# roryclear/clearcam

Hardware: AMD Instinct MI355X
Metric: yolov9c_640x640_frames_per_sec (higher is better)
Workload: dtype f16; 1 GPU; YOLOv9-C f16h batch=64 640x640 frames (letterbox 640) per GPU, uint8 BGR frames resident in HBM, seeded synthetic weights, full detect path (letterbox+convs+decode+top300+NMS); batch_per_gpu=64, parallelism=one camera batch per GPU x1, no collective, batches_in_flight=3

## Files before the change

clearcam_amd/csrc/conv_direct.hip:

```cpp
#include "kernels.h"

namespace cc {

template <class T>
__global__ __launch_bounds__(256) void conv_direct_kernel(const ConvP p) {
  const size_t total = (size_t)p.B * p.Ho * p.Wo * p.Cout;
  const size_t idx = (size_t)blockIdx.x * 256 + threadIdx.x;
  if (idx >= total) return;
  const int n = (int)(idx % p.Cout);
  const size_t m = idx / p.Cout;
  const int hw = p.Ho * p.Wo;
  const int b = (int)(m / hw), rem = (int)(m - (size_t)b * hw), ho = rem / p.Wo, wo = rem - ho * p.Wo;
  const T* w = reinterpret_cast<const T*>(p.w) + (size_t)n * p.Kw;
  float acc = 0.f;
  for (int r = 0; r < p.ks; ++r) {
    const int ih = ho * p.stride - p.pad + r;
    if ((unsigned)ih >= (unsigned)p.Hin) continue;
    for (int s = 0; s < p.ks; ++s) {
      const int iw = wo * p.stride - p.pad + s;
      if ((unsigned)iw >= (unsigned)p.Win) continue;
      for (int h = 0; h <= p.split; ++h) {
        const T* wk = w + ((r * p.ks + s) * (1 + p.split) + h) * p.Cin;
        {
          const Src& S = p.s0;
// ... 159 lines not shown

template <class T>
__global__ __launch_bounds__(256) void avgmax_rows2_kernel(const PoolP p) {
  constexpr int E = 16 / (int)sizeof(T);
  const int CV = p.C / E;
  const int x = blockIdx.x * 256 + threadIdx.x;
  if (x >= p.Wo * CV) return;
  const int wo = x / CV, cv = x - wo * CV, ho0 = blockIdx.y * 2, b = blockIdx.z;
  const T* in = reinterpret_cast<const T*>(p.in) + p.in_coff + cv * E;
  const int i0 = 2 * ho0 - 1, j0 = 2 * wo - 1;
  uint4 u[6][4];
#pragma unroll
  for (int r = 0; r < 6; ++r) {
    const int ic = min(max(i0 + r, 0), p.H - 1);
#pragma unroll
    for (int c = 0; c < 4; ++c) {
      const int jc = min(max(j0 + c, 0), p.W - 1);
      u[r][c] = *reinterpret_cast<const uint4*>(in + ((size_t)(b * p.H + ic) * p.W + jc) * p.in_cstride);
    }
  }
#pragma unroll
  for (int q = 0; q < 2; ++q) {
    const int ho = ho0 + q;
    if (ho >= p.Ho) break;
    float acc[E];
#pragma unroll
    for (int e = 0; e < E; ++e) acc[e] = -INFINITY;
#pragma unroll
    for (int r = 0; r < 3; ++r) {
      const int ph = i0 + 2 * q + r;
      float top[4][E], bot[4][E];
#pragma unroll
      for (int c = 0; c < 4; ++c) { unpack_chunk<T>(u[2 * q + r][c], top[c]); unpack_chunk<T>(u[2 * q + r + 1][c], bot[c]); }
#pragma unroll
      for (int s = 0; s < 3; ++s) {
        const int pw = j0 + s;
        const bool ok = ph >= 0 && ph <= p.H - 2 && pw >= 0 && pw <= p.W - 2;
#pragma unroll
        for (int e = 0; e < E; ++e) {
          const float a = (((top[s][e] + top[s + 1][e]) + bot[s][e]) + bot[s + 1][e]) * 0.25f;
          acc[e] = fmaxf(acc[e], ok ? a : -INFINITY);
        }
      }
    }
    uint4 o;
    T* t = reinterpret_cast<T*>(&o);
#pragma unroll
    for (int e = 0; e < E; ++e) t[e] = from_f32<T>(acc[e]);
    const size_t m = ((size_t)b * p.Ho + ho) * p.Wo + wo;
    *reinterpret_cast<uint4*>(reinterpret_cast<T*>(p.out) + m * p.out_cstride + p.out_coff + cv * E) = o;
  }
}

template <class T>
__global__ __launch_bounds__(256) void pool_kernel(const PoolP p) {
  const size_t total = (size_t)p.B * p.Ho * p.Wo * p.C;
  const size_t idx = (size_t)blockIdx.x * 256 + threadIdx.x;
  if (idx >= total) return;
  const int c = (int)(idx % p.C);
  const size_t m = idx / p.C;
  const int hw = p.Ho * p.Wo;
  const int b = (int)(m / hw), rem = (int)(m - (size_t)b * hw), ho = rem / p.Wo, wo = rem - ho * p.Wo;
  const T* in = reinterpret_cast<const T*>(p.in);
  float acc = p.mode ? -INFINITY : 0.f;
  for (int r = 0; r < p.k; ++r) {
    const int ih = ho * p.stride - p.pad + r;
    if ((unsigned)ih >= (unsigned)p.H) continue;
    for (int s = 0; s < p.k; ++s) {
      const int iw = wo * p.stride - p.pad + s;
      if ((unsigned)iw >= (unsigned)p.W) continue;
      const float v = to_f32<T>(in[((size_t)(b * p.H + ih) * p.W + iw) * p.in_cstride + p.in_coff + c]);
      acc = p.mode ? fmaxf(acc, v) : acc + v;
    }
  }
  if (!p.mode) acc = acc * (1.0f / (float)(p.k * p.k));
  reinterpret_cast<T*>(p.out)[m * p.out_cstride + p.out_coff + c] = from_f32<T>(acc);
}

std::atomic<int> g_pool_rows_override{-1};
constexpr int kNoPoolRows = INT32_MIN;
static int pool_rows() {
  const int ov = g_pool_rows_override.load();
  if (ov >= 0) return ov;
  static const int env = [] { const char* e = getenv("CLEARCAM_POOL_ROWS"); return e ? atoi(e) : kNoPoolRows; }();
  return env;
}

PoolKernel choose_pool(int dt, const PoolP& p) {
  const int E = dt == F32 ? 4 : 8;
  const bool vec = p.C % E == 0 && p.in_coff % E == 0 && p.in_cstride % E == 0 && p.out_coff % E == 0 && p.out_cstride % E == 0 &&
                   ((uintptr_t)p.in & 15) == 0 && ((uintptr_t)p.out & 15) == 0;
  const int set = pool_rows();
  if (p.mode == 2) {
    CC_CHECK(vec && p.k == 3 && p.stride == 2 && p.pad == 1, "avg-max pool: needs 16-byte channel chunks, k=3 s=2 p=1");
    const int rows2 = set == kNoPoolRows ? 4 : set;
    return rows2 != 1 && p.Ho >= 32 ? POOL_AVGMAX_ROWS2 : POOL_AVGMAX;
  }
  if (vec && p.mode == 0 && p.k == 2) {
    const int rows = set == kNoPoolRows ? 8 : set;
    const bool plain = p.stride == 1 && p.pad == 0 && p.Ho >= 64 && p.Wo == p.W - 1 && p.Ho == p.H - 1;
    if (rows == 8 && plain) return POOL_AVG2_ROWS8;
    if (rows == 4 && plain) return POOL_AVG2_ROWS4;
    return POOL_VEC_AVG2;
  }
  if (vec && p.mode == 1 && p.k == 1) return POOL_VEC_MAX1;
  if (vec && p.mode == 1 && p.k == 2) return POOL_VEC_MAX2;
  if (vec && p.mode == 1 && p.k == 3) return POOL_VEC_MAX3;
  if (vec && p.mode == 1 && p.k == 5) return POOL_VEC_MAX5;
  return POOL_SCALAR;
}

template <class T> static void launch_pool_t(PoolKernel k, const PoolP& p, hipStream_t stream) {
  constexpr int E = 16 / (int)sizeof(T);
  const dim3 vgrid((unsigned)((p.Wo * (p.C / E) + 255) / 256), (unsigned)p.Ho, (unsigned)p.B);
  auto rows_grid = [&](int r) { return dim3(vgrid.x, (unsigned)((p.Ho + r - 1) / r), vgrid.z); };
  switch (k) {
    case POOL_AVGMAX_ROWS2: hipLaunchKernelGGL(avgmax_rows2_kernel<T>, rows_grid(2), dim3(256), 0, stream, p); break;
    case POOL_AVGMAX: hipLaunchKernelGGL(avgmax_pool_kernel<T>, vgrid, dim3(256), 0, stream, p); break;
    case POOL_AVG2_ROWS8: hipLaunchKernelGGL((avg2_rows_kernel<T, 8>), rows_grid(8), dim3(256), 0, stream, p); break;
    case POOL_AVG2_ROWS4: hipLaunchKernelGGL((avg2_rows_kernel<T, 4>), rows_grid(4), dim3(256), 0, stream, p); break;
    case POOL_VEC_AVG2: hipLaunchKernelGGL((pool_vec_kernel<T, 2, 0>), vgrid, dim3(256), 0, stream, p); break;
    case POOL_VEC_MAX1: hipLaunchKernelGGL((pool_vec_kernel<T, 1, 1>), vgrid, dim3(256), 0, stream, p); break;
    case POOL_VEC_MAX2: hipLaunchKernelGGL((pool_vec_kernel<T, 2, 1>), vgrid, dim3(256), 0, stream, p); break;
    case POOL_VEC_MAX3: hipLaunchKernelGGL((pool_vec_kernel<T, 3, 1>), vgrid, dim3(256), 0, stream, p); break;
    case POOL_VEC_MAX5: hipLaunchKernelGGL((pool_vec_kernel<T, 5, 1>), vgrid, dim3(256), 0, stream, p); break;
    case POOL_SCALAR: {
      const size_t total = (size_t)p.B * p.Ho * p.Wo * p.C;
      hipLaunchKernelGGL(pool_kernel<T>, dim3((unsigned)((total + 255) / 256)), dim3(256), 0, stream, p);
      break;
    }
  }
  CC_HIP(hipGetLastError());
}

template <class T>
__global__ __launch_bounds__(256) void fuse_kernel(const FuseP p) {
  constexpr int E = 16 / (int)sizeof(T);
  const int CV = p.C / E;
  const size_t total = (size_t)p.B * p.Ho * p.Wo * CV;
  const size_t idx = (size_t)blockIdx.x * 256 + threadIdx.x;
  if (idx >= total) return;
  const int cv = (int)(idx % CV);
  const size_t m = idx / CV;
  const int hw = p.Ho * p.Wo;
  const int b = (int)(m / hw), rem = (int)(m - (size_t)b * hw), ho = rem / p.Wo, wo = rem - ho * p.Wo;
  float acc[E];
#pragma unroll
  for (int e = 0; e < E; ++e) acc[e] = 0.f;
  for (int k = 0; k < p.n; ++k) {
    const T* in = reinterpret_cast<const T*>(p.in[k]) +
                  ((size_t)(b * p.H[k] + (ho >> p.shift[k])) * p.W[k] + (wo >> p.shift[k])) * p.cstride[k] + p.coff[k] + cv * E;
    const uint4 u = *reinterpret_cast<const uint4*>(in);
    const T* t = reinterpret_cast<const T*>(&u);
#pragma unroll
    for (int e = 0; e < E; ++e) acc[e] += to_f32<T>(t[e]);
  }
  uint4 o;
  T* t = reinterpret_cast<T*>(&o);
#pragma unroll
  for (int e = 0; e < E; ++e) t[e] = from_f32<T>(acc[e]);
  *reinterpret_cast<uint4*>(reinterpret_cast<T*>(p.out) + m * p.out_cstride + p.out_coff + cv * E) = o;
}

void launch_fuse(int dt, const FuseP& p, hipStream_t stream) {
  const int E = dt == F32 ? 4 : 8;
  CC_CHECK(p.C % E == 0 && p.out_coff % E == 0 && p.out_cstride % E == 0, "fuse: channel alignment");
  for (int k = 0; k < p.n; ++k) CC_CHECK(p.coff[k] % E == 0 && p.cstride[k] % E == 0, "fuse: input channel alignment");
  const size_t total = (size_t)p.B * p.Ho * p.Wo * (p.C / E);
  const dim3 grid((unsigned)((total + 255) / 256)), block(256);
// ... 16 lines not shown
```

clearcam_amd/csrc/dev_glue.hip:

```cpp
#include "conv_select.h"
#include "yolo_plan.h"

using namespace cc;

namespace {

bool aligned16(const void* p) { return (reinterpret_cast<uintptr_t>(p) & 15u) == 0; }
constexpr long kMaxElems = 1L << 30;

PoolP pool_args(int dtype, const void* in_dev, int in_cstride, int in_coff, void* out_dev, int out_cstride, int out_coff, int B, int H, int W,
                int C, int Ho, int Wo, int k, int stride, int pad, int mode) {
  CC_CHECK(dtype == F32 || dtype == F16 || dtype == BF16, "dtype must be 0 (f32), 1 (f16) or 2 (bf16)");
  CC_CHECK(in_dev && out_dev, "null argument");
  CC_CHECK(B > 0 && H > 0 && W > 0 && C > 0 && Ho > 0 && Wo > 0, "bad shape");
  CC_CHECK(mode >= 0 && mode <= 2 && k > 0 && k <= 16 && stride > 0 && pad >= 0 && pad < k, "bad window");
  CC_CHECK(in_coff >= 0 && in_coff + C <= in_cstride && out_coff >= 0 && out_coff + C <= out_cstride, "bad channel view");
  CC_CHECK((long)B * H * W * in_cstride < kMaxElems && (long)B * Ho * Wo * out_cstride < kMaxElems, "tensor too large");
  const int Hp = mode == 2 ? H - 1 : H, Wp = mode == 2 ? W - 1 : W;
  CC_CHECK(Hp > 0 && Wp > 0, "avg-max pool: the input needs two rows and two columns");
  if (mode == 0) CC_CHECK(pad == 0 && (Ho - 1) * stride + k <= H && (Wo - 1) * stride + k <= W, "avg pool: windows must lie inside the input (pad 0)");
  else CC_CHECK((Ho - 1) * stride - pad < Hp && (Wo - 1) * stride - pad < Wp, "Ho / Wo beyond the padded input");
  PoolP p{};
  p.in = in_dev; p.in_cstride = in_cstride; p.in_coff = in_coff; p.out = out_dev; p.out_cstride = out_cstride; p.out_coff = out_coff;
  p.B = B; p.H = H; p.W = W; p.C = C; p.Ho = Ho; p.Wo = Wo; p.k = k; p.stride = stride; p.pad = pad; p.mode = mode;
  return p;
}

Src src_view(const cc_src_desc& s) { return Src{s.ptr, s.H, s.W, s.cstride, s.coff, s.C, s.shift}; }

int dev_conv(bool det, bool launch, const cc_conv_desc* d, const cc_src_desc* s0, const cc_src_desc* s1, const float* w_oihw, const float* bias,
             const void* res_dev, void* out_dev, int* choice, void* stream) {
  PackedConv pc;
  auto release = [&]() { if (pc.w) hipFree(pc.w); if (pc.bias) hipFree(pc.bias); pc.w = nullptr; pc.bias = nullptr; };
  try {
    CC_CHECK(d && s0 && out_dev && (w_oihw || !launch), "null argument");
    CC_CHECK(d->dtype == F32 || d->dtype == F16 || d->dtype == BF16 || d->dtype == F16S, "dtype must be 0 (f32), 1 (f16), 2 (bf16) or 3 (f16s)");
    const int split = d->dtype == F16S, dt = storage_dtype(d->dtype);
    CC_CHECK(d->B > 0 && d->H > 0 && d->W > 0 && d->k > 0 && d->k <= 7 && d->stride > 0 && d->Cin > 0 && d->Cout > 0, "bad shape");
    if (!det) CC_CHECK(d->groups == 1 && d->act >= 0 && d->act <= 2 && !d->res_f32 && !d->res_cstride && !d->res_coff, "one group, act 0 .. 2, no residual");
    else {
      CC_CHECK(d->groups >= 1 && d->Cin % d->groups == 0 && d->Cout % d->groups == 0, "groups must divide Cin and Cout");
      CC_CHECK(d->act >= 0 && d->act <= (launch ? 2 : 4), "act 0 .. 2");
      CC_CHECK(res_dev || (!d->res_f32 && !d->res_cstride && !d->res_coff), "a residual view without a residual pointer");
    }
    ConvP c{};
    c.s0 = src_view(*s0);
    c.s1 = s1 ? src_view(*s1) : Src{s0->ptr, 1, 1, 0, 0, 0, 0};
    c.B = d->B; c.Hin = d->H; c.Win = d->W; c.Cin = d->Cin; c.Cout = d->Cout; c.ks = d->k; c.stride = d->stride; c.pad = d->pad < 0 ? d->k / 2 : d->pad;
    c.Ho = d->Ho > 0 ? d->Ho : (c.Hin + 2 * c.pad - c.ks) / c.stride + 1; c.Wo = d->Wo > 0 ? d->Wo : (c.Win + 2 * c.pad - c.ks) / c.stride + 1;
    CC_CHECK(c.s0.C > 0 && c.s1.C >= 0 && c.s0.C + c.s1.C == c.Cin, "Cin must be the channels of the two sources");
    for (const Src* s : {&c.s0, &c.s1}) {
      if (s->C == 0) continue;
      CC_CHECK(s->ptr && s->H > 0 && s->W > 0 && s->coff >= 0 && s->coff + s->C <= s->cstride && (long)c.B * s->H * s->W * s->cstride < kMaxElems, "bad source view");
      CC_CHECK(s->shift >= -1 && s->shift <= 4, "shift must be -1 (2x2 average), 0 or a nearest-upsample exponent");
      if (s->shift >= 0) CC_CHECK(((c.Hin - 1) >> s->shift) < s->H && ((c.Win - 1) >> s->shift) < s->W, "a source is smaller than the input over 2^shift");
      else CC_CHECK(s == &c.s0 && c.Hin == s->H - 1 && c.Win == s->W - 1, "the 2x2 average: first source only, input = (H - 1) x (W - 1) of it");
    }
    c.out = out_dev; c.out_cstride = d->out_cstride > 0 ? d->out_cstride : d->Cout; c.out_coff = d->out_coff; c.out_f32 = d->out_f32 ? 1 : 0;
    c.act = d->act; c.variant = d->variant; c.split = split;
    c.Ktot = c.ks * c.ks * c.Cin * (1 + split);
    c.Kw = (c.Ktot + 63) / 64 * 64;
    CC_CHECK(c.Ho > 0 && c.Wo > 0 && c.out_coff >= 0 && c.out_coff + c.Cout <= c.out_cstride && (long)c.B * c.Ho * c.Wo * c.out_cstride < kMaxElems, "bad output view");
    CC_CHECK(c.pad >= 0 && c.pad < c.ks && (c.Ho - 1) * c.stride - c.pad < c.Hin && (c.Wo - 1) * c.stride - c.pad < c.Win, "Ho / Wo beyond the padded input");
    const bool adown = c.s0.shift < 0;
    if (res_dev) {
      c.res = res_dev; c.res_f32 = d->res_f32 ? 1 : 0; c.res_cstride = d->res_cstride > 0 ? d->res_cstride : d->Cout; c.res_coff = d->res_coff;
      CC_CHECK(c.res_coff >= 0 && c.res_coff + c.Cout <= c.res_cstride && (long)c.B * c.Ho * c.Wo * c.res_cstride < kMaxElems, "bad residual view");
      CC_CHECK(!adown, "the averaging loader takes no residual");
      CC_CHECK(res_dev != out_dev || (c.res_f32 == c.out_f32 && c.res_cstride == c.out_cstride && c.res_coff == c.out_coff),
// ... 93 lines not shown
```

clearcam_amd/csrc/kernels.h:

```cpp
#pragma once
#include <atomic>
#include <vector>
#include "common.h"

namespace cc {

struct LaunchNote { const char* kernel; long tiles; long slots; };
extern thread_local LaunchNote g_launch_note;
extern thread_local bool g_note_launches;
template <class K> inline void note_launch(const char* name, K kernel, long tiles, int threads, size_t lds, long persistent_grid = 0) {
  if (!g_note_launches) return;
  long slots = persistent_grid;
  if (!slots) {
    int nb = 0;
    if (hipOccupancyMaxActiveBlocksPerMultiprocessor(&nb, reinterpret_cast<const void*>(kernel), threads, lds) != hipSuccess) nb = 1;
    slots = (long)nb * cu_count();
  }
  g_launch_note = LaunchNote{name, tiles, slots > 0 ? slots : 1};
}

bool conv_mfma_supported(int dt, const ConvP& p);
void launch_conv_mfma(int dt, const ConvP& p, hipStream_t stream);
void launch_conv_direct(int dt, const ConvP& p, hipStream_t stream);
void launch_conv(int dt, const ConvP& p, hipStream_t stream);
bool conv_adown_supported(int dt, const ConvP& p);
int conv_adown_bn(const ConvP& p);
void launch_conv_adown(int dt, const ConvP& p, hipStream_t stream);

struct CspP {
  const void* x; int x_cstride, x_coff;
  void* out; int out_cstride, out_coff;
  const void* w12; int kw12; const float* b12;
  const void* wr; int kwr; const float* br;
  const void* wb; int kwb; const float* bb;
  const void* w3; int kw3; const float* b3;
  int B, H, W, hid;
  int split; float os12, osr, osb, os3;
  int tx, tiles; float inv_tiles, inv_tx;
  int dbg;
  int stream;
};
bool csp_fused_supported(int dt, int hid, int split = 0);
enum CspKernel : int { CSP_FUSED_RESIDENT = 0, CSP_FUSED_STREAMED = 1, CSP_TILE = 2 };
CspKernel choose_csp(int dt, int hid, int split, int B, int H, int W, int stream, int dbg, int tile_mode);
extern std::atomic<int> g_csp_tile_override;
int csp_tile_mode();
void launch_csp_fused(int dt, const CspP& p, hipStream_t stream, CspKernel* chosen = nullptr);

void launch_sample_rows(const ConvP& p, const int* rows_dev, int S, float* out_dev, hipStream_t stream);
void second_moments(const float* X, int rows, int ci, std::vector<double>& H);
int gptq_round_f16(const float* w, int co, int ci, const double* H, double damp, float* out);

struct PoolP {
  const void* in; int in_cstride, in_coff;
  void* out; int out_cstride, out_coff;
  int B, H, W, C;
  int Ho, Wo;
  int k, stride, pad;
  int mode;
};
enum PoolKernel : int {
  POOL_SCALAR = 0,
  POOL_VEC_MAX1 = 1,
  POOL_VEC_MAX2 = 2,
  POOL_VEC_MAX3 = 3,
  POOL_VEC_MAX5 = 4,
  POOL_VEC_AVG2 = 5,
  POOL_AVG2_ROWS4 = 6,
  POOL_AVG2_ROWS8 = 7,
  POOL_AVGMAX = 8,
  POOL_AVGMAX_ROWS2 = 9,
};
PoolKernel choose_pool(int dt, const PoolP& p);
extern std::atomic<int> g_pool_rows_override;
void launch_pool(int dt, const PoolP& p, hipStream_t stream, PoolKernel* chosen = nullptr);

struct FuseP {
  int n;
  const void* in[6]; int H[6], W[6], cstride[6], coff[6], shift[6];
  void* out; int out_cstride, out_coff;
  int B, Ho, Wo, C;
};
void launch_fuse(int dt, const FuseP& p, hipStream_t stream);

struct PreP {
  const void* frames; int frame_f32;
  int B, H, W;
  int nh, nw, pad_y, pad_x, Hn, Wn;
  const int* xlo; const int* xhi; const float* xfr;
  const int* ylo; const int* yhi; const float* yfr;
  void* out; int out_c;
  int flip;
  float div, sub, pad_val;
};
void launch_preprocess(int dt, const PreP& p, hipStream_t stream);

struct FrameDesc {
  long long off;
  int H, W, nh, nw, pad_y, pad_x;
  const int* xlo; const int* xhi; const float* xfr;
  const int* ylo; const int* yhi; const float* yfr;
  float fpad_x, fpad_y, gain, src_w, src_h;
  int reserved;
};
void launch_preprocess_ragged(int dt, const PreP& p, const FrameDesc* desc, size_t packed_bytes, hipStream_t stream);

struct StemP {
  PreP pre;
  const void* w; const float* bias;
  const void* w_lo; float oscale;
  int Cout;
  void* out; int out_cstride, out_coff;
  int Ho, Wo;
  int abl;
};
bool stem_fused_supported(int dt, int Cout);
void stem_pack_weights(int dt, const void* w_packed, int w_row, int tap_stride, int plane_off, int Cout, void* out, hipStream_t stream);
void launch_stem_fused(int dt, const StemP& p, hipStream_t stream);
bool stem_needs_big(int H, int W, int nh, int nw, int frame_f32);
void launch_stem_fused_ragged(int dt, const StemP& p, const FrameDesc* desc, size_t packed_bytes, bool big, hipStream_t stream);
void axis_tables(int n_in, int n_out, std::vector<int>& lo, std::vector<int>& hi, std::vector<float>& fr);

struct DecodeP {
  const float* raw[3]; int H[3], W[3];
  int B, A;
  const float* dfl_w;
  float conf;
// ... 173 lines not shown
```

clearcam_amd/csrc/yolo.hip:

```cpp
#include <cmath>
#include <cstring>
#include "conv_select.h"
#include "yolo_plan.h"

using namespace cc;

namespace cc {

static const Arch kArch[] = {
    {"t", 16, true, 32, 32, false, 64, 16, 64, 64, 96, 24, 96, 128, 32, 128, 64, 48, 64, 80, 3},
    {"s", 32, true, 64, 64, false, 128, 32, 128, 128, 192, 48, 192, 256, 64, 256, 128, 96, 128, 128, 3},
    {"m", 32, false, 32, 128, false, 240, 60, 240, 240, 360, 90, 360, 480, 120, 480, 240, 184, 240, 240, 1},
    {"c", 64, false, 32, 256, true, 256, 64, 256, 512, 512, 128, 512, 512, 128, 512, 256, 256, 512, 256, 1},
    {"e", 64, false, 32, 256, true, 0, 0, 256, 0, 0, 0, 512, 0, 0, 512, 256, 0, 0, 256, 2},
};

void convert_f32_to(int dt, const float* src, void* dst, size_t n) {
  if (dt == F32) memcpy(dst, src, n * 4);
  else if (dt == F16) { f16_t* d = (f16_t*)dst; for (size_t i = 0; i < n; ++i) d[i] = (f16_t)src[i]; }
  else { uint16_t* d = (uint16_t*)dst; for (size_t i = 0; i < n; ++i) d[i] = f32_to_bf16_bits(src[i]); }
}

static int weight_rounding() {
  static const int mode = [] {
// ... 93 lines not shown
  const int cp = cin_pad > cin ? cin_pad : cin;
  const int planes = split ? 2 : 1;
  const size_t kreal = (size_t)k * k * cp * planes;
  const size_t ktot = (kreal + 63) / 64 * 64;
  std::vector<float> w((size_t)cout * ktot, 0.f), bias(cout, 0.f);
  float scale = 1.0f;
  if (split) {
    float mx = 0.f;
    for (size_t t = 0; t < ws.size(); ++t) for (float v : ws[t]->data) mx = std::max(mx, std::fabs(v));
    if (mx > 0.f && std::isfinite(mx)) scale = std::ldexp(1.0f, 14 - std::ilogb(mx));
    pc.split = 1; pc.oscale = 1.0f / scale;
  }
  int n0 = 0;
  for (size_t t = 0; t < ws.size(); ++t) {
    const int co = (int)ws[t]->shape[0], cig = (int)ws[t]->shape[1], g = groups[t], cog = co / g;
    pc.macs_px += (double)co * cig * k * k;
    std::vector<float> fb;
    if (!split && dt != F32 && weight_rounding() != 0) fb = round_weights(dt, *ws[t]);
    const float* src = fb.empty() ? ws[t]->data.data() : fb.data();
    for (int n = 0; n < co; ++n) {
      const int grp = n / cog;
      for (int c = 0; c < cig; ++c)
        for (int r = 0; r < k; ++r)
          for (int s = 0; s < k; ++s) {
            const float v = src[(((size_t)n * cig + c) * k + r) * k + s];
            float* row = &w[(size_t)(n0 + n) * ktot];
            if (!split) row[(size_t)(r * k + s) * cp + grp * cig + c] = v;
            else {
              const float vs = v * scale;
              const float hi = (float)(f16_t)vs;
              row[(size_t)((r * k + s) * 2 + 0) * cp + grp * cig + c] = hi;
              row[(size_t)((r * k + s) * 2 + 1) * cp + grp * cig + c] = vs - hi;
            }
          }
      if (bs[t]) bias[n0 + n] = bs[t]->data[n];
    }
    n0 += co;
  }
  std::vector<char> tmp(w.size() * dtype_size(dt));
  convert_f32_to(dt, w.data(), tmp.data(), w.size());
  CC_HIP(hipMalloc(&pc.w, tmp.size() + 256));
  CC_HIP(hipMemcpy(pc.w, tmp.data(), tmp.size(), hipMemcpyHostToDevice));
  CC_HIP(hipMalloc((void**)&pc.bias, cout * 4));
  CC_HIP(hipMemcpy(pc.bias, bias.data(), cout * 4, hipMemcpyHostToDevice));
  pc.cin = cp; pc.cout = cout; pc.k = k; pc.kw = (int)ktot;
  return pc;
}

struct PlanSwitches {
  static int num(const char* name, int dflt) { const char* e = getenv(name); return e ? atoi(e) : dflt; }
  static bool set(const char* name) { return getenv(name) != nullptr; }
  const int lanes = num("CLEARCAM_LANES", 0), fuse_csp = num("CLEARCAM_FUSE_CSP", 2);
  const bool fuse_stem = num("CLEARCAM_FUSE_STEM", 1) != 0, fuse_adown = num("CLEARCAM_FUSE_ADOWN", 0) != 0, fuse_head = num("CLEARCAM_FUSE_HEAD", 1) != 0;
  const bool head_split = num("CLEARCAM_HEAD_SPLIT", 1) != 0, arena_reuse = num("CLEARCAM_ARENA_REUSE", 1) != 0;
  const bool tap_csp = set("CLEARCAM_TAP_CSP"), tap_stem = set("CLEARCAM_TAP_STEM"), tap_blocks = set("CLEARCAM_TAP_BLOCKS"), verbose = set("CLEARCAM_VERBOSE");
  const bool dev = num("CLEARCAM_DEV", 0) != 0;
  const bool csp_only_set = dev && set("CLEARCAM_CSP_ONLY");
  const int csp_only = dev ? num("CLEARCAM_CSP_ONLY", 0) : 0, csp_dbg = dev ? num("CLEARCAM_CSP_DBG", 0) : 0, csp_stream = dev ? num("CLEARCAM_CSP_STREAM", 0) : 0;
};

struct Builder {
  cc_yolo* Y; Plan* P; const Arch& a; const PlanSwitches sw;
  Builder(cc_yolo* y, Plan* p) : Y(y), P(p), a(*y->arch) {}

  int cur_lane = 0;
  struct Lane {
    Builder& b; int saved;
    Lane(Builder& b_, int l) : b(b_), saved(b_.cur_lane) {
      const int m = b.sw.lanes;
      if (l == 1 ? (m & 1) : (m & 6)) b.cur_lane = (l > 2 && (m & 4)) ? 2 : l;
    }
    ~Lane() { b.cur_lane = saved; }
  };
  static Op::Access rd(View v) { return Op::Access{v.buf, v.coff, v.C, false}; }
  static Op::Access wr(View v) { return Op::Access{v.buf, v.coff, v.C, true}; }
  void push(Op& op, std::vector<Op::Access> acc) { op.lane = cur_lane; op.acc = std::move(acc); P->ops.push_back(op); }

  int new_buf(int H, int W, int C, bool f32 = false) {
    Buf b{H, W, C, f32, P->arena_bytes};
    size_t bytes = (size_t)P->B * H * W * C * (f32 ? 4 : dtype_size(Y->dtype));
    P->arena_bytes += (bytes + 255) & ~(size_t)255;
    P->bufs.push_back(b);
    return (int)P->bufs.size() - 1;
  }
  View whole(int buf) { return View{buf, 0, P->bufs[buf].C}; }
  static View slice(View v, int c0, int C) { return View{v.buf, v.coff + c0, C}; }

  static int block_of(const std::string& name) {
    const size_t at = name.find("model.list.");
    CC_CHECK(at == 0 && isdigit((unsigned char)name[11]), "conv parameter outside model.list.<block>: " + name);
    return atoi(name.c_str() + 11);
  }
  const PackedConv& pconv(const std::vector<std::string>& names, const std::vector<int>& groups, int cin_pad = 0) {
    std::string key;
    for (auto& n : names) key += n + "+";
    auto it = Y->packed.find(key);
    if (it != Y->packed.end()) return it->second;
    std::vector<const HostTensor*> ws, bs;
    for (auto& n : names) {
      auto w = Y->host.find(n + ".weight");
      CC_CHECK(w != Y->host.end(), "missing parameter " + n + ".weight");
      auto b = Y->host.find(n + ".bias");
      CC_CHECK(b != Y->host.end(), "missing parameter " + n + ".bias");
      ws.push_back(&w->second); bs.push_back(&b->second);
    }
    const int blk = block_of(names[0]);
    const bool k1 = ws[0]->shape.size() == 4 && ws[0]->shape[2] == 1;
// ... 151 lines not shown

  View elan1(const std::string& p, View in, int hid, int cout) {
    const int H = P->bufs[in.buf].H, W = P->bufs[in.buf].W;
    const int cat = new_buf(H, W, 2 * hid), o = new_buf(H, W, cout);
    conv({{in, 0}}, pconv({p + ".cv1.conv"}, {1}), slice(whole(cat), 0, hid), 1, 1);
    conv({{slice(whole(cat), hid / 2, hid / 2), 0}}, pconv({p + ".cv2.conv"}, {1}), slice(whole(cat), hid, hid / 2), 1, 1);
    conv({{slice(whole(cat), hid, hid / 2), 0}}, pconv({p + ".cv3.conv"}, {1}), slice(whole(cat), hid + hid / 2, hid / 2), 1, 1);
    conv({{whole(cat), 0}}, pconv({p + ".cv4.conv"}, {1}), whole(o), 1, 1);
    return whole(o);
  }

  bool fuse_adown(View in) const {
    if (!sw.fuse_adown || Y->wsplit) return false;
    return Y->dtype != F32 && in.C % 64 == 0 && in.coff % 8 == 0 && P->bufs[in.buf].C % 8 == 0;
  }
  View down(const std::string& p, View in, int cout) {
    const int H = P->bufs[in.buf].H, W = P->bufs[in.buf].W, C = in.C;
    const int Ho = (H - 1 + 2 - 3) / 2 + 1, Wo = (W - 1 + 2 - 3) / 2 + 1;
    const int o = new_buf(Ho, Wo, cout);
    if (a.adown) {
      CC_CHECK(C == cout, "ADown keeps the channel count");
      {
        Lane lane(*this, 1);
        const int mp = new_buf(Ho, Wo, C / 2);
        const int E = Y->dtype == F32 ? 4 : 8;
        if ((C / 2) % E == 0 && in.coff % E == 0 && P->bufs[in.buf].C % E == 0) {
          pool(slice(in, C / 2, C / 2), whole(mp), 3, 2, 1, 2);
        } else {
          const int avg2 = new_buf(H - 1, W - 1, C / 2);
          pool(slice(in, C / 2, C / 2), whole(avg2), 2, 1, 0, 0);
          pool(whole(avg2), whole(mp), 3, 2, 1, 1);
        }
        conv({{whole(mp), 0}}, pconv({p + ".cv2.conv"}, {1}), slice(whole(o), C / 2, C / 2), 1, 1);
      }
      if (fuse_adown(slice(in, 0, C / 2))) {
        conv({{slice(in, 0, C / 2), -1}}, pconv({p + ".cv1.conv"}, {1}), slice(whole(o), 0, C / 2), 2, 1);
      } else {
        const int avg = new_buf(H - 1, W - 1, C / 2);
        pool(slice(in, 0, C / 2), whole(avg), 2, 1, 0, 0);
        conv({{whole(avg), 0}}, pconv({p + ".cv1.conv"}, {1}), slice(whole(o), 0, C / 2), 2, 1);
      }
    } else {
      const int avg = new_buf(H - 1, W - 1, C);
      pool(in, whole(avg), 2, 1, 0, 0);
      conv({{whole(avg), 0}}, pconv({p + ".cv1.conv"}, {1}), whole(o), 2, 1);
    }
    return whole(o);
  }

  View sppelan(const std::string& p, View in, int hid, int cout) {
    const int H = P->bufs[in.buf].H, W = P->bufs[in.buf].W;
    const int cat = new_buf(H, W, 4 * hid), o = new_buf(H, W, cout);
    conv({{in, 0}}, pconv({p + ".cv1.conv"}, {1}), slice(whole(cat), 0, hid), 1, 1);
    for (int i = 0; i < 3; ++i) pool(slice(whole(cat), i * hid, hid), slice(whole(cat), (i + 1) * hid, hid), 5, 1, 2, 1);
    conv({{whole(cat), 0}}, pconv({p + ".cv5.conv"}, {1}), whole(o), 1, 1);
    return whole(o);
  }

  View cblinear(const std::string& p, View in) {
    const PackedConv& pc = pconv({p + ".conv"}, {1});
    const int o = new_buf(P->bufs[in.buf].H, P->bufs[in.buf].W, pc.cout);
    conv({{in, 0}}, pc, whole(o), 1, 0);
    return whole(o);
  }
  View cbfuse(const std::vector<View>& parts, View last) {
    const Buf& lb = P->bufs[last.buf];
    const int o = new_buf(lb.H, lb.W, last.C);
    Op op{}; op.kind = Fuse; FuseP& f = op.fuse;
    f.n = (int)parts.size() + 1; CC_CHECK(f.n <= 6, "CBFuse: too many inputs");
    for (int k = 0; k < f.n; ++k) {
      const View& v = k + 1 < f.n ? parts[k] : last;
      const Buf& b = P->bufs[v.buf];
      CC_CHECK(v.C == last.C && lb.H % b.H == 0, "CBFuse input mismatch");
      int sh = 0; while ((b.H << sh) < lb.H) ++sh;
      CC_CHECK((b.H << sh) == lb.H && (b.W << sh) == lb.W, "CBFuse scale must be a power of two");
      f.in[k] = (const void*)(intptr_t)v.buf; f.H[k] = b.H; f.W[k] = b.W; f.cstride[k] = b.C; f.coff[k] = v.coff; f.shift[k] = sh;
    }
    f.out = (void*)(intptr_t)o; f.out_cstride = last.C; f.out_coff = 0; f.B = P->B; f.Ho = lb.H; f.Wo = lb.W; f.C = last.C;
    std::vector<Op::Access> acc{wr(whole(o)), rd(last)};
    for (const View& v : parts) acc.push_back(rd(v));
    push(op, std::move(acc));
    return whole(o);
  }

  bool fuse_head_tail() const {
    return sw.fuse_head && head_tail_supported(Y->dtype, a.cls_hidden, Y->wsplit);
  }
  Op head_dec{}, head_tail{};
  std::vector<Op::Access> head_acc;
  int head_levels = 0;
  void head_level(const std::string& H22, int l, View feat) {
    Lane lane(*this, 2 + l);
    const bool fused = fuse_head_tail();
    if (head_levels++ == 0) { head_dec = Op{}; head_dec.kind = Decode; head_tail = Op{}; head_tail.kind = HeadTail; head_acc.clear(); P->A = 0; }
    const std::string hb = H22 + "cv2.list." + std::to_string(l) + ".list.", hc = H22 + "cv3.list." + std::to_string(l) + ".list.";
    const int H = P->bufs[feat.buf].H, W = P->bufs[feat.buf].W, ch = a.cls_hidden;
    const int hbuf = new_buf(H, W, 64 + ch), bxb = new_buf(H, W, 64), clb = new_buf(H, W, ch);
    if (sw.head_split && Y->dtype != F32 && ch % 256 == 0) {
      conv({{feat, 0}}, pconv({hb + "0.conv"}, {1}), slice(whole(hbuf), 0, 64), 1, 1);
      conv({{feat, 0}}, pconv({hc + "0.conv"}, {1}), slice(whole(hbuf), 64, ch), 1, 1);
    } else
    conv({{feat, 0}}, pconv({hb + "0.conv", hc + "0.conv"}, {1, 1}), whole(hbuf), 1, 1);
    conv({{slice(whole(hbuf), 0, 64), 0}}, pconv({hb + "1.conv"}, {4}), whole(bxb), 1, 1);
    conv({{slice(whole(hbuf), 64, ch), 0}}, pconv({hc + "1.conv"}, {1}), whole(clb), 1, 1);
    const PackedConv &c2 = pconv({hb + "2"}, {4}), &c3 = pconv({hc + "2"}, {1});
    if (fused) {
      CC_CHECK(c2.cin == 64 && c2.cout == 64 && c2.k == 1 && c3.cin == ch && c3.cout == 80 && c3.k == 1, "fused DDetect tail: unexpected conv shapes");
// ... 295 lines not shown
```

clearcam_amd/csrc/yolo_profile.hip:

```cpp
#include <cstring>
#include "yolo_plan.h"

using namespace cc;

static std::string op_kind_name(const Op& op) {
  switch (op.kind) {
    case Conv: return op.conv.s0.shift < 0 ? "conv_avg" : "conv";
    case Pool: return "pool" + std::to_string(op.pool.mode) + "_k" + std::to_string(op.pool.k) + "_s" + std::to_string(op.pool.stride);
    case Decode: return "decode";      case Nms: return "topk_nms";     case Fuse: return "cbfuse";
    case Stem: return "stem_fused";    case Csp: return "csp_fused";    case HeadTail: return "head_tail";
  }
  return "";
}
static int profile_slot(OpKind k) {
  switch (k) {
    case Conv: case Csp: return 0;
    case Pool: case Fuse: return 1;
    case Decode: case HeadTail: return 2;
    case Nms: return 3;
    case Stem: return 4;
  }
  return 0;
}

// ... 91 lines not shown
  double acc[5] = {0, 0, 0, 0, 0}, macs = 0; int nconv = 0;
  std::vector<cc::LaunchNote> notes(n, cc::LaunchNote{"", 0, 1});
  if (getenv("CLEARCAM_PROFILE_CSV")) {
    for (size_t i = 0; i < n; ++i) {
      cc::g_note_launches = true;
      cc::g_launch_note = cc::LaunchNote{"", 0, 1};
      launch_op(h->dtype, P, P->ops[i], s, true);
      notes[i] = cc::g_launch_note;
      cc::g_note_launches = false;
    }
    CC_HIP(hipStreamSynchronize(s));
  }
  for (int it = 0; it < iters; ++it) {
    for (size_t i = 0; i < n; ++i) {
      const Op& op = P->ops[i];
      CC_HIP(hipEventRecord(ev[2 * i], s));
      launch_op(h->dtype, P, op, s, true);
      CC_HIP(hipEventRecord(ev[2 * i + 1], s));
    }
    CC_HIP(hipStreamSynchronize(s));
    for (size_t i = 0; i < n; ++i) {
      float t = 0; CC_HIP(hipEventElapsedTime(&t, ev[2 * i], ev[2 * i + 1]));
      acc[profile_slot(P->ops[i].kind)] += t;
    }
  }
  for (const Op& op : P->ops) if (op.kind == Conv || op.kind == Csp) { macs += op.alg_macs; ++nconv; }
  if (const char* path = getenv("CLEARCAM_PROFILE_CSV")) {
    FILE* f = fopen(path, "w");
    if (f) {
      fprintf(f, "op,kind,ms,M,Cout,Ktot,ks,stride,Cin,alg_gmac,tflops,gbytes_min,gbs,weight_planes,kernel,tiles,slots,rounds,last_round_fill,bound,roof_ms\n");
      auto tail = [&](size_t i, double macs, double bytes) {
        const cc::LaunchNote& ln = notes[i];
        const long rounds = ln.tiles ? (ln.tiles + ln.slots - 1) / ln.slots : 0;
        const double fill = rounds ? (double)(ln.tiles - (rounds - 1) * ln.slots) / (double)ln.slots : 0.0;
        const double tm = 2 * macs / 2.5e15 * 1e3, tb = bytes / 8e12 * 1e3;
        fprintf(f, ",%s,%ld,%ld,%ld,%.3f,%s,%.4f\n", ln.kernel, ln.tiles, ln.slots, rounds, fill, tm > tb ? "mfma" : "hbm", tm > tb ? tm : tb);
      };
      for (size_t i = 0; i < n; ++i) {
        const Op& op = P->ops[i];
        float t = 0; hipEventElapsedTime(&t, ev[2 * i], ev[2 * i + 1]);
        const std::string kind = op_kind_name(op);
        if (op.kind == Conv) {
          const ConvP& c = op.conv; const double M = (double)c.B * c.Ho * c.Wo;
          const double es = dtype_size(h->dtype);
          const bool avg = c.s0.shift < 0;
          const double in0 = avg ? (double)(c.Hin + 1) * (c.Win + 1) : (double)(c.Hin >> c.s0.shift) * (c.Win >> c.s0.shift);
          const double bytes = (double)c.B * in0 * c.s0.C * es + (double)c.B * (c.Hin >> c.s1.shift) * (c.Win >> c.s1.shift) * c.s1.C * es
                             + M * c.Cout * (c.out_f32 ? 4 : es) + (c.res ? M * c.Cout * es : 0) + (double)c.Cout * c.Ktot * es;
          fprintf(f, "%zu,%s,%.4f,%.0f,%d,%d,%d,%d,%d,%.4f,%.1f,%.4f,%.0f,%d", i, kind.c_str(), t, M, c.Cout, c.Ktot, c.ks, c.stride, c.Cin,
                  op.alg_macs / 1e9, 2 * op.alg_macs / (t * 1e-3) / 1e12, bytes / 1e9, bytes / (t * 1e-3) / 1e9, 1 + c.split);
          tail(i, op.alg_macs, bytes);
        } else if (op.kind == Pool) {
          const PoolP& q = op.pool; const double es = dtype_size(h->dtype);
          const double bytes = ((double)q.B * q.H * q.W + (double)q.B * q.Ho * q.Wo) * q.C * es;
          fprintf(f, "%zu,%s,%.4f,%.0f,%d,0,%d,%d,%d,0,0,%.4f,%.0f,0", i, kind.c_str(), t, (double)q.B * q.Ho * q.Wo, q.C, q.k, q.stride, q.C,
                  bytes / 1e9, bytes / (t * 1e-3) / 1e9);
          tail(i, 0.0, bytes);
        } else if (op.kind == Stem) {
          const StemP& q = op.stem; const double M = (double)q.pre.B * q.Ho * q.Wo, es = dtype_size(h->dtype);
          const double bytes = (double)q.pre.B * q.pre.H * q.pre.W * 3 * (q.pre.frame_f32 ? 4 : 1) + M * q.Cout * es;
          fprintf(f, "%zu,%s,%.4f,%.0f,%d,27,3,2,3,%.4f,%.1f,%.4f,%.0f,%d", i, kind.c_str(), t, M, q.Cout, op.alg_macs / 1e9, 2 * op.alg_macs / (t * 1e-3) / 1e12,
                  bytes / 1e9, bytes / (t * 1e-3) / 1e9, q.w_lo ? 2 : 1);
          tail(i, op.alg_macs, bytes);
        } else if (op.kind == Csp) {
          const CspP& q = op.csp; const double M = (double)q.B * q.H * q.W, es = dtype_size(h->dtype);
          const double bytes = M * 4 * q.hid * es + (double)(8 + 18) * q.hid * q.hid * es;
          fprintf(f, "%zu,%s,%.4f,%.0f,%d,%d,3,1,%d,%.4f,%.1f,%.4f,%.0f,%d", i, kind.c_str(), t, M, 2 * q.hid, (8 + 18) * q.hid, 2 * q.hid, op.alg_macs / 1e9,
                  2 * op.alg_macs / (t * 1e-3) / 1e12, bytes / 1e9, bytes / (t * 1e-3) / 1e9, q.split ? 2 : 1);
          tail(i, op.alg_macs, bytes);
        } else fprintf(f, "%zu,%s,%.4f,0,0,0,0,0,0,0,0,0,0,0,,0,0,0,0,,0\n", i, kind.c_str(), t);
      }
      fclose(f);
    }
  }
  for (auto& e : ev) hipEventDestroy(e);
  for (int k = 0; k < 5; ++k) ms[k] = (float)(acc[k] / iters);
  if (alg_macs_per_step) *alg_macs_per_step = macs;
  if (n_conv_launches) *n_conv_launches = nconv;
  CC_API_END
}

int cc_yolo_profile_graph(cc_yolo* h, int iters, int which, float* ms_per_replay) {
  CC_API_BEGIN
  CC_CHECK(h && ms_per_replay && h->last && iters > 0 && which >= 0 && which <= 2, "bad argument / no detect call yet");
  Plan* P = h->last;
  CC_CHECK(!P->ragged, "cc_yolo_profile_graph: the last call was a ragged batch - profile the uniform plan of the same network shape");
  CC_HIP(hipSetDevice(h->device));
  hipStream_t s = h->stream;
  sync_all(h);
  hipGraph_t graph = nullptr; hipGraphExec_t exec = nullptr;
  CC_HIP(hipStreamBeginCapture(s, hipStreamCaptureModeThreadLocal));
  try {
    for (const Op& op : P->ops) {
      const bool conv = op.kind == Conv || op.kind == Csp;
      if (which == 0 ? !conv : (which == 1 ? conv : false)) continue;
      launch_op(h->dtype, P, op, s, true);
    }
  } catch (...) { hipStreamEndCapture(s, &graph); if (graph) hipGraphDestroy(graph); throw; }
  CC_HIP(hipStreamEndCapture(s, &graph));
  CC_HIP(hipGraphInstantiate(&exec, graph, nullptr, nullptr, 0));
  CC_HIP(hipGraphDestroy(graph));
  for (int i = 0; i < 2; ++i) CC_HIP(hipGraphLaunch(exec, s));
  CC_HIP(hipEventRecord(h->ev0, s));
  for (int i = 0; i < iters; ++i) CC_HIP(hipGraphLaunch(exec, s));
  CC_HIP(hipEventRecord(h->ev1, s));
  CC_HIP(hipEventSynchronize(h->ev1));
  float t = 0; CC_HIP(hipEventElapsedTime(&t, h->ev0, h->ev1));
// ... 7 lines not shown
```

Before: 6539 frames/s.

## Fuse SPPELAN's three chained max pools into one LDS-resident kernel

Adds a pool mode that loads the SPP input map once into LDS and applies three separable 5x5 max pools in sequence, writing each result to its slice of the concat buffer. This replaces three separate pool launches, which each re-read the previous output from global memory. The cost is LDS use that limits the map to at most 2048 pixels, and a grid of only channel-groups times batch blocks, which may leave occupancy low.

Measured after the change: 6568 frames/s (median of 6 runs). About the same (+0.4%).

```diff
diff --git a/clearcam_amd/csrc/conv_direct.hip b/clearcam_amd/csrc/conv_direct.hip
--- a/clearcam_amd/csrc/conv_direct.hip
+++ b/clearcam_amd/csrc/conv_direct.hip
@@ -235,6 +235,69 @@
   }
 }
 
+template <class T> __device__ inline uint4 chunk_max(const uint4& a, const uint4& b) {
+  constexpr int E = 16 / (int)sizeof(T);
+  float x[E], y[E];
+  unpack_chunk<T>(a, x); unpack_chunk<T>(b, y);
+  uint4 o;
+  T* t = reinterpret_cast<T*>(&o);
+#pragma unroll
+  for (int e = 0; e < E; ++e) t[e] = from_f32<T>(fmaxf(x[e], y[e]));
+  return o;
+}
+typedef _Float16 f16x2_t __attribute__((ext_vector_type(2)));
+template <> __device__ inline uint4 chunk_max<f16_t>(const uint4& a, const uint4& b) {
+  union { uint4 u; f16x2_t h[4]; } x, y, o;
+  x.u = a; y.u = b;
+#pragma unroll
+  for (int i = 0; i < 4; ++i) o.h[i] = __builtin_elementwise_max(x.h[i], y.h[i]);
+  return o.u;
+}
+
+constexpr int kSppLdsBytes = 64 * 1024;
+template <class T, int G>
+__global__ __launch_bounds__(256) void spp3_kernel(const PoolP p) {
+  constexpr int E = 16 / (int)sizeof(T);
+  extern __shared__ uint4 spp_lds[];
+  const int HW = p.H * p.W, n = HW * G;
+  uint4* A = spp_lds;
+  uint4* Rm = spp_lds + n;
+  const int CV = p.C / E, b = blockIdx.y, g = threadIdx.x % G;
+  const int cv = blockIdx.x * G + g;
+  const bool live = cv < CV;
+  const T* in = reinterpret_cast<const T*>(p.in) + (size_t)b * HW * p.in_cstride + p.in_coff + cv * E;
+  T* out = reinterpret_cast<T*>(p.out) + (size_t)b * HW * p.out_cstride + p.out_coff + cv * E;
+  for (int i = threadIdx.x; i < n; i += 256)
+    A[i] = live ? *reinterpret_cast<const uint4*>(in + (size_t)(i / G) * p.in_cstride) : uint4{0u, 0u, 0u, 0u};
+  __syncthreads();
+  for (int k = 0; k < 3; ++k) {
+    for (int i = threadIdx.x; i < n; i += 256) {
+      const int pix = i / G, y = pix / p.W, xx = pix - y * p.W;
+      uint4 m = A[i];
+#pragma unroll
+      for (int d = -2; d <= 2; ++d)
+        if (d) m = chunk_max<T>(m, A[(y * p.W + min(max(xx + d, 0), p.W - 1)) * G + g]);
+      Rm[i] = m;
+    }
+    __syncthreads();
+    for (int i = threadIdx.x; i < n; i += 256) {
+      const int pix = i / G, y = pix / p.W, xx = pix - y * p.W;
+      uint4 m = Rm[i];
+#pragma unroll
+      for (int d = -2; d <= 2; ++d)
+        if (d) m = chunk_max<T>(m, Rm[(min(max(y + d, 0), p.H - 1) * p.W + xx) * G + g]);
+      A[i] = m;
+      if (live) *reinterpret_cast<uint4*>(out + (size_t)pix * p.out_cstride + k * p.C) = m;
+    }
+    __syncthreads();
+  }
+}
+static int spp3_group(const PoolP& p) {
+  const long hw = (long)p.H * p.W;
+  for (int g = 4; g >= 1; g >>= 1) if (hw * g * 32 <= kSppLdsBytes) return g;
+  return 0;
+}
+
 template <class T>
 __global__ __launch_bounds__(256) void pool_kernel(const PoolP p) {
   const size_t total = (size_t)p.B * p.Ho * p.Wo * p.C;
@@ -269,11 +332,22 @@
   return env;
 }
 
+static bool pool_chunks_ok(int dt, const PoolP& p) {
+  const int E = dt == F32 ? 4 : 8;
+  return p.C % E == 0 && p.in_coff % E == 0 && p.in_cstride % E == 0 && p.out_coff % E == 0 && p.out_cstride % E == 0;
+}
+static bool pool_vec_ok(int dt, const PoolP& p) { return pool_chunks_ok(dt, p) && ((uintptr_t)p.in & 15) == 0 && ((uintptr_t)p.out & 15) == 0; }
+bool spp3_supported(int dt, const PoolP& p) {
+  return p.mode == 3 && p.k == 5 && p.stride == 1 && p.pad == 2 && p.Ho == p.H && p.Wo == p.W && pool_chunks_ok(dt, p) && spp3_group(p) > 0;
+}
+
 PoolKernel choose_pool(int dt, const PoolP& p) {
-  const int E = dt == F32 ? 4 : 8;
-  const bool vec = p.C % E == 0 && p.in_coff % E == 0 && p.in_cstride % E == 0 && p.out_coff % E == 0 && p.out_cstride % E == 0 &&
-                   ((uintptr_t)p.in & 15) == 0 && ((uintptr_t)p.out & 15) == 0;
+  const bool vec = pool_vec_ok(dt, p);
   const int set = pool_rows();
+  if (p.mode == 3) {
+    CC_CHECK(vec && spp3_supported(dt, p), "chained max pools: needs 16-byte channel chunks, k=5 s=1 p=2 and a map of at most 2048 pixels");
+    return POOL_SPP3;
+  }
   if (p.mode == 2) {
     CC_CHECK(vec && p.k == 3 && p.stride == 2 && p.pad == 1, "avg-max pool: needs 16-byte channel chunks, k=3 s=2 p=1");
     const int rows2 = set == kNoPoolRows ? 4 : set;
@@ -298,6 +372,15 @@
   const dim3 vgrid((unsigned)((p.Wo * (p.C / E) + 255) / 256), (unsigned)p.Ho, (unsigned)p.B);
   auto rows_grid = [&](int r) { return dim3(vgrid.x, (unsigned)((p.Ho + r - 1) / r), vgrid.z); };
   switch (k) {
+    case POOL_SPP3: {
+      const int g = spp3_group(p);
+      const dim3 grid((unsigned)((p.C / E + g - 1) / g), (unsigned)p.B);
+      const size_t lds = (size_t)p.H * p.W * g * 32;
+      if (g == 4) hipLaunchKernelGGL((spp3_kernel<T, 4>), grid, dim3(256), lds, stream, p);
+      else if (g == 2) hipLaunchKernelGGL((spp3_kernel<T, 2>), grid, dim3(256), lds, stream, p);
+      else hipLaunchKernelGGL((spp3_kernel<T, 1>), grid, dim3(256), lds, stream, p);
+      break;
+    }
     case POOL_AVGMAX_ROWS2: hipLaunchKernelGGL(avgmax_rows2_kernel<T>, rows_grid(2), dim3(256), 0, stream, p); break;
     case POOL_AVGMAX: hipLaunchKernelGGL(avgmax_pool_kernel<T>, vgrid, dim3(256), 0, stream, p); break;
     case POOL_AVG2_ROWS8: hipLaunchKernelGGL((avg2_rows_kernel<T, 8>), rows_grid(8), dim3(256), 0, stream, p); break;
diff --git a/clearcam_amd/csrc/dev_glue.hip b/clearcam_amd/csrc/dev_glue.hip
--- a/clearcam_amd/csrc/dev_glue.hip
+++ b/clearcam_amd/csrc/dev_glue.hip
@@ -13,8 +13,14 @@
   CC_CHECK(dtype == F32 || dtype == F16 || dtype == BF16, "dtype must be 0 (f32), 1 (f16) or 2 (bf16)");
   CC_CHECK(in_dev && out_dev, "null argument");
   CC_CHECK(B > 0 && H > 0 && W > 0 && C > 0 && Ho > 0 && Wo > 0, "bad shape");
-  CC_CHECK(mode >= 0 && mode <= 2 && k > 0 && k <= 16 && stride > 0 && pad >= 0 && pad < k, "bad window");
-  CC_CHECK(in_coff >= 0 && in_coff + C <= in_cstride && out_coff >= 0 && out_coff + C <= out_cstride, "bad channel view");
+  CC_CHECK(mode >= 0 && mode <= 3 && k > 0 && k <= 16 && stride > 0 && pad >= 0 && pad < k, "bad window");
+  const int Cw = mode == 3 ? 3 * C : C;
+  CC_CHECK(in_coff >= 0 && in_coff + C <= in_cstride && out_coff >= 0 && out_coff + Cw <= out_cstride, "bad channel view");
+  if (mode == 3) {
+    CC_CHECK(k == 5 && stride == 1 && pad == 2 && Ho == H && Wo == W, "chained max pools: k=5 s=1 p=2 on the input's own grid");
+    CC_CHECK(in_dev != out_dev || (in_cstride == out_cstride && (in_coff + C <= out_coff || out_coff + Cw <= in_coff)),
+             "chained max pools in place: the input channels must lie outside the three output slices");
+  }
   CC_CHECK((long)B * H * W * in_cstride < kMaxElems && (long)B * Ho * Wo * out_cstride < kMaxElems, "tensor too large");
   const int Hp = mode == 2 ? H - 1 : H, Wp = mode == 2 ? W - 1 : W;
   CC_CHECK(Hp > 0 && Wp > 0, "avg-max pool: the input needs two rows and two columns");
diff --git a/clearcam_amd/csrc/kernels.h b/clearcam_amd/csrc/kernels.h
--- a/clearcam_amd/csrc/kernels.h
+++ b/clearcam_amd/csrc/kernels.h
@@ -70,9 +70,11 @@
   POOL_AVG2_ROWS8 = 7,
   POOL_AVGMAX = 8,
   POOL_AVGMAX_ROWS2 = 9,
+  POOL_SPP3 = 10,
 };
 PoolKernel choose_pool(int dt, const PoolP& p);
 extern std::atomic<int> g_pool_rows_override;
+bool spp3_supported(int dt, const PoolP& p);
 void launch_pool(int dt, const PoolP& p, hipStream_t stream, PoolKernel* chosen = nullptr);
 
 struct FuseP {
diff --git a/clearcam_amd/csrc/yolo.hip b/clearcam_amd/csrc/yolo.hip
--- a/clearcam_amd/csrc/yolo.hip
+++ b/clearcam_amd/csrc/yolo.hip
@@ -169,7 +169,7 @@
   static bool set(const char* name) { return getenv(name) != nullptr; }
   const int lanes = num("CLEARCAM_LANES", 0), fuse_csp = num("CLEARCAM_FUSE_CSP", 2);
   const bool fuse_stem = num("CLEARCAM_FUSE_STEM", 1) != 0, fuse_adown = num("CLEARCAM_FUSE_ADOWN", 0) != 0, fuse_head = num("CLEARCAM_FUSE_HEAD", 1) != 0;
-  const bool head_split = num("CLEARCAM_HEAD_SPLIT", 1) != 0, arena_reuse = num("CLEARCAM_ARENA_REUSE", 1) != 0;
+  const bool head_split = num("CLEARCAM_HEAD_SPLIT", 1) != 0, arena_reuse = num("CLEARCAM_ARENA_REUSE", 1) != 0, fuse_spp = num("CLEARCAM_FUSE_SPP", 1) != 0;
   const bool tap_csp = set("CLEARCAM_TAP_CSP"), tap_stem = set("CLEARCAM_TAP_STEM"), tap_blocks = set("CLEARCAM_TAP_BLOCKS"), verbose = set("CLEARCAM_VERBOSE");
   const bool dev = num("CLEARCAM_DEV", 0) != 0;
   const bool csp_only_set = dev && set("CLEARCAM_CSP_ONLY");
@@ -427,7 +427,14 @@
     const int H = P->bufs[in.buf].H, W = P->bufs[in.buf].W;
     const int cat = new_buf(H, W, 4 * hid), o = new_buf(H, W, cout);
     conv({{in, 0}}, pconv({p + ".cv1.conv"}, {1}), slice(whole(cat), 0, hid), 1, 1);
-    for (int i = 0; i < 3; ++i) pool(slice(whole(cat), i * hid, hid), slice(whole(cat), (i + 1) * hid, hid), 5, 1, 2, 1);
+    Op sp{}; sp.kind = Pool; PoolP& q = sp.pool;
+    q.in = q.out = (void*)(intptr_t)cat; q.in_cstride = q.out_cstride = 4 * hid; q.in_coff = 0; q.out_coff = hid;
+    q.B = P->B; q.H = q.Ho = H; q.W = q.Wo = W; q.C = hid; q.k = 5; q.stride = 1; q.pad = 2; q.mode = 3;
+    if (sw.fuse_spp && spp3_supported(Y->dtype, q)) {
+      push(sp, {rd(slice(whole(cat), 0, hid)), wr(slice(whole(cat), hid, hid)), wr(slice(whole(cat), 2 * hid, hid)), wr(slice(whole(cat), 3 * hid, hid))});
+    } else {
+      for (int i = 0; i < 3; ++i) pool(slice(whole(cat), i * hid, hid), slice(whole(cat), (i + 1) * hid, hid), 5, 1, 2, 1);
+    }
     conv({{whole(cat), 0}}, pconv({p + ".cv5.conv"}, {1}), whole(o), 1, 1);
     return whole(o);
   }
diff --git a/clearcam_amd/csrc/yolo_profile.hip b/clearcam_amd/csrc/yolo_profile.hip
--- a/clearcam_amd/csrc/yolo_profile.hip
+++ b/clearcam_amd/csrc/yolo_profile.hip
@@ -167,7 +167,7 @@
           tail(i, op.alg_macs, bytes);
         } else if (op.kind == Pool) {
           const PoolP& q = op.pool; const double es = dtype_size(h->dtype);
-          const double bytes = ((double)q.B * q.H * q.W + (double)q.B * q.Ho * q.Wo) * q.C * es;
+          const double bytes = ((double)q.B * q.H * q.W + (double)q.B * q.Ho * q.Wo * (q.mode == 3 ? 3 : 1)) * q.C * es;
           fprintf(f, "%zu,%s,%.4f,%.0f,%d,0,%d,%d,%d,0,0,%.4f,%.0f,0", i, kind.c_str(), t, (double)q.B * q.Ho * q.Wo, q.C, q.k, q.stride, q.C,
                   bytes / 1e9, bytes / (t * 1e-3) / 1e9);
           tail(i, 0.0, bytes);
```
